# osqp/miosqp

Hardware: AMD Instinct MI355X
Metric: ADMM iterations/s (random_miqp n=500 m=1000 p=250, node-at-a-time B&B) (higher is better)
Workload: dtype f64

## Files before the change

include/miosqp_amd.h:

```cpp
#ifndef MIOSQP_AMD_H
#define MIOSQP_AMD_H

#include <stdint.h>

#ifdef __cplusplus
extern "C" {
#endif

#define MIOSQP_QP_SOLVED 1
#define MIOSQP_QP_MAX_ITER_REACHED (-2)
#define MIOSQP_QP_PRIMAL_INFEASIBLE (-3)
#define MIOSQP_QP_DUAL_INFEASIBLE (-4)
#define MIOSQP_QP_UNSOLVED (-10)

#define MIOSQP_EARG (-1)
#define MIOSQP_EHIP (-2)
#define MIOSQP_EFACTOR (-3)
#define MIOSQP_ENODEV (-4)
#define MIOSQP_EUNSUPPORTED (-5)
#define MIOSQP_EFULL (-6)
#define MIOSQP_EBOUNDS 1

typedef struct miosqp_qp_settings {
  double rho;
// ... 430 lines not shown
                                         double *x_out, miosqp_tree_info *info, miosqp_lockstep_stats *stats,
                                         miosqp_lockstep_ahead_stats *ahead_stats);

typedef struct miosqp_search_info {
  int64_t nodes;
  int64_t osqp_iter;
  int32_t open_leaves;
  int32_t free_slots;
  int32_t improved;
  int32_t reserved;
  double upper_glob, lower_glob;
  double device_time;
  double run_time;
} miosqp_search_info;

int miosqp_qp_search_create(miosqp_qp_engine *e, int32_t capacity);
int miosqp_qp_search_reset(miosqp_qp_engine *e);
int miosqp_qp_search_add_leaf(miosqp_qp_engine *e, const double *l_int, const double *u_int, const double *x0,
                              const double *y0, int32_t depth, double lower);
int miosqp_qp_search_take_leaf(miosqp_qp_engine *e, double *l_int, double *u_int, double *x0, double *y0,
                               int32_t *depth, double *lower);
int miosqp_qp_search_set_incumbent(miosqp_qp_engine *e, double upper, const double *x);
int miosqp_qp_search_get_incumbent(miosqp_qp_engine *e, double *upper, double *x);
int miosqp_qp_search_run(miosqp_qp_engine *e, int32_t tree_explor_rule, int64_t max_nodes, double budget_s,
                         miosqp_search_info *info);

typedef struct miosqp_pool_digest {
  int32_t slot;
  int32_t status_val;
  int32_t iter;
  int32_t int_inf;
  int32_t nextvar;
  int32_t reserved;
  double lower;
  double heur_viol;
  double heur_obj;
  double pri_res, dua_res;
} miosqp_pool_digest;

int miosqp_qp_pool_create(miosqp_qp_engine *e, int32_t capacity, int32_t columns);
int miosqp_qp_pool_reset(miosqp_qp_engine *e);
int miosqp_qp_pool_write_node(miosqp_qp_engine *e, int32_t slot, const double *l_int, const double *u_int,
                              const double *x0, const double *y0);
int miosqp_qp_pool_read_node(miosqp_qp_engine *e, int32_t slot, double *l_int, double *u_int, double *x, double *y);
int miosqp_qp_pool_push(miosqp_qp_engine *e, int32_t count, const int32_t *slot, const int32_t *child0,
                        const int32_t *child1, const double *lower);
// ... 66 lines not shown
```

miosqp_amd/_lib.py:

```python
import ctypes as C
import os

_PKG = os.path.dirname(os.path.abspath(__file__))
LIB_PATH = os.path.join(_PKG, "libmiosqp_hip.so")

dp = C.POINTER(C.c_double)
dpp = C.POINTER(dp)
ip = C.POINTER(C.c_int32)
i64p = C.POINTER(C.c_int64)


class Settings(C.Structure):
    _fields_ = [(k, C.c_double) for k in
                ("rho", "sigma", "alpha", "eps_abs", "eps_rel", "eps_prim_inf", "eps_dual_inf")] + \
               [(k, C.c_int32) for k in ("max_iter", "scaling", "check_termination", "warm_start",
                                         "device", "max_batch", "fold", "resident", "setup_on_device", "coop", "pers", "batch_pers",
                                         "rho_auto")]


class Info(C.Structure):
    _fields_ = [("status_val", C.c_int32), ("iter", C.c_int32), ("run_time", C.c_double),
                ("obj_val", C.c_double), ("pri_res", C.c_double), ("dua_res", C.c_double),
                ("device_time", C.c_double), ("lower", C.c_double),
                ("int_inf", C.c_int32), ("nextvar", C.c_int32), ("heur_viol", C.c_double),
# ... 189 lines not shown
    "miosqp_qp_setup_group": (C.c_int64, [C.c_void_p]),
    "miosqp_qp_debug_product_form": (C.c_int, [C.c_void_p, C.c_int32, dp, C.c_int64, ip, ip]),
    "miosqp_qp_solve_trees_lockstep": (C.c_int, [C.c_void_p, C.c_int32, dp, dp, dp, dp, dp, dp, dp, C.c_int32, C.c_int32,
                                                 C.c_int32, dp, C.POINTER(TreeInfo), C.POINTER(LockstepStats)]),
    "miosqp_qp_solve_trees_lockstep_rf": (C.c_int, [C.c_void_p, C.c_int32, dp, dp, dp, dp, dp, dp, dp, C.c_int32, C.c_int32,
                                                    C.c_int32, C.c_int32, C.c_int32, C.c_int32, dp, C.POINTER(TreeInfo),
                                                    C.POINTER(LockstepStats), C.POINTER(LockstepRfStats)]),
    "miosqp_qp_solve_trees_lockstep_sb": (C.c_int, [C.c_void_p, C.c_int32, dp, dp, dp, dp, dp, dp, dp, C.c_int32, C.c_int32,
                                                    C.c_int32, C.c_int32, C.c_int32, C.c_int32, C.c_int32, C.c_double, dp,
                                                    C.POINTER(TreeInfo), C.POINTER(LockstepStats),
                                                    C.POINTER(LockstepSbStats)]),
    "miosqp_qp_solve_trees_lockstep_ahead": (C.c_int, [C.c_void_p, C.c_int32, dp, dp, dp, dp, dp, dp, dp, C.c_int32,
                                                       C.c_int32, C.c_int32, C.c_int32, dp, C.POINTER(TreeInfo),
                                                       C.POINTER(LockstepStats), C.POINTER(LockstepAheadStats)]),
    "miosqp_qp_solve_trees_refill": (C.c_int, [C.c_void_p, C.c_int32, dp, dp, dp, dp, dp, dp, dp, C.c_int32, C.c_int32,
                                               C.c_int32, dp, C.POINTER(TreeInfo), C.POINTER(RefillStats)]),
    "miosqp_qp_search_create": (C.c_int, [C.c_void_p, C.c_int32]),
    "miosqp_qp_search_reset": (C.c_int, [C.c_void_p]),
    "miosqp_qp_search_add_leaf": (C.c_int, [C.c_void_p, dp, dp, dp, dp, C.c_int32, C.c_double]),
    "miosqp_qp_search_take_leaf": (C.c_int, [C.c_void_p, dp, dp, dp, dp, C.POINTER(C.c_int32), C.POINTER(C.c_double)]),
    "miosqp_qp_search_set_incumbent": (C.c_int, [C.c_void_p, C.c_double, dp]),
    "miosqp_qp_search_get_incumbent": (C.c_int, [C.c_void_p, C.POINTER(C.c_double), dp]),
    "miosqp_qp_search_run": (C.c_int, [C.c_void_p, C.c_int32, C.c_int64, C.c_double, C.POINTER(SearchInfo)]),
    "miosqp_qp_stream_create": (C.c_int, [C.c_void_p, C.c_int32, C.c_int32, C.c_int32]),
    "miosqp_qp_stream_begin": (C.c_int, [C.c_void_p]),
    "miosqp_qp_stream_add_leaf": (C.c_int, [C.c_void_p, dp, dp, dp, dp, C.c_int32, C.c_double]),
    "miosqp_qp_stream_take_leaf": (C.c_int, [C.c_void_p, dp, dp, dp, dp, C.POINTER(C.c_int32), C.POINTER(C.c_double)]),
    "miosqp_qp_stream_set_incumbent": (C.c_int, [C.c_void_p, C.c_double, dp]),
    "miosqp_qp_stream_get_incumbent": (C.c_int, [C.c_void_p, C.POINTER(C.c_double), dp]),
    "miosqp_qp_stream_step": (C.c_int, [C.c_void_p, C.c_int32, C.c_int32, C.c_int32, C.c_int64, C.POINTER(StreamInfo)]),
    "miosqp_qp_solve_batch": (C.c_int, [C.c_void_p, C.c_int32, dp, dp, dp, dp, dp, dp,
                                        C.POINTER(Info)]),
    "miosqp_qp_solve_batch_q": (C.c_int, [C.c_void_p, C.c_int32, dp, dp, dp, dp, dp, dp, dp,
                                          C.POINTER(Info)]),
    "miosqp_qp_solve_tree": (C.c_int, [C.c_void_p, dp, dp, dp, dp, C.c_double, dp, C.c_int32, C.c_int32, dp,
                                       C.POINTER(TreeInfo)]),
    "miosqp_qp_pool_create": (C.c_int, [C.c_void_p, C.c_int32, C.c_int32]),
    "miosqp_qp_pool_reset": (C.c_int, [C.c_void_p]),
    "miosqp_qp_pool_write_node": (C.c_int, [C.c_void_p, C.c_int32, dp, dp, dp, dp]),
    "miosqp_qp_pool_read_node": (C.c_int, [C.c_void_p, C.c_int32, dp, dp, dp, dp]),
    "miosqp_qp_pool_push": (C.c_int, [C.c_void_p, C.c_int32, ip, ip, ip, dp]),
    "miosqp_qp_pool_set_upper": (C.c_int, [C.c_void_p, C.c_double]),
    "miosqp_qp_pool_launch": (C.c_int, [C.c_void_p, C.c_int32]),
    "miosqp_qp_pool_collect": (C.c_int, [C.c_void_p, C.c_int32, C.POINTER(PoolDigest), C.c_int32, C.POINTER(C.c_int32),
                                         C.POINTER(C.c_int32), i64p]),
    "miosqp_qp_cleanup": (C.c_int, [C.c_void_p]),
# ... 61 lines not shown
```

miosqp_amd/csrc/engine.hip:

```cpp
#include <hip/hip_runtime.h>

#include <dlfcn.h>
#include <sys/stat.h>

#include <algorithm>
#include <chrono>
#include <cmath>
#include <cstdio>
#include <cstdlib>
#include <cstring>
#include <map>
#include <mutex>
#include <queue>
#include <deque>
#include <tuple>
#include <type_traits>
#include <string>
#include <vector>

#include "../../include/miosqp_amd.h"
#include "factor.hpp"
#include "polish_many.hpp"
#include "polish_many_large.hpp"
#include "lockstep_trees.hpp"
// ... 76 lines not shown
  double *sm, *sn;
  double *raw_l, *raw_u, *raw_x, *raw_y, *out_x, *out_y;
  Ctrl *ctrl;
  const double *f_rows, *f_GmT, *f_Ad, *f_Atd, *f_Pd;
  int ldf, ldn, ldm;
  double *rx;
  double *xi, *xis, *root_l, *root_u;
  double eps_int, eps_lin;
  int digest;
  int bm_ablate;
  unsigned long long *prof;
  const double *W;
  int ldw;
  unsigned *coop_tag;
  unsigned long long *coop_buf;
  unsigned long long *coop_chk;
  unsigned long long *coop_q;
  unsigned long long *coop_reg;
  unsigned long long *coop_chz;
  unsigned long long *coop_dec;
  int coop_nt;
  int coop_lag;
  int coop_tres;
  const double *Kc;
  int coop_dbg;
  int coop_nap;
  int coop_stride;
  size_t coop_half;
  const double *coop_W;
  int coop_ldw, coop_mg;
  const int *coop_brow;
  const double *coop_aj;
  int Bs;
  double *b_l, *b_u, *b_x, *b_z, *b_y, *b_wh, *b_rx, *b_cv, *b_ut, *b_xt, *b_dx, *b_dy;
  double *b_xfs;
  double *b_sm, *b_sn;
  double *b_xfin, *b_yfin;
  double *b_xi, *b_xis;
  double *b_part;
  const double *b_zero;
  int stream;
  int max_iter_s, ring;
  int *c_start, *c_child0, *c_child1, *c_harv, *t_has;
  int *fmap, *hmap;
  double *lt_x;
  const int *int_pos;
// ... 2573 lines not shown
```

miosqp_amd/csrc/host.inc:

```
constexpr int POOL_EVENTS = 8;
constexpr int COOP_RETRY = -1000;

inline int pick_tpr(double avg_row) {
  if (avg_row <= 48) return 16;
  if (avg_row <= 192) return 32;
  if (avg_row <= 640) return 64;
  if (avg_row <= 1536) return 128;
  return 256;
}

#define DISPATCH_TPR(tpr, KERNEL, rows, stream, ...)                                              \
  do {                                                                                            \
    switch (tpr) {                                                                                \
      case 16: hipLaunchKernelGGL(KERNEL<16>, dim3(((rows) + 15) / 16), dim3(256), 0, stream, __VA_ARGS__); break;   \
      case 32: hipLaunchKernelGGL(KERNEL<32>, dim3(((rows) + 7) / 8), dim3(256), 0, stream, __VA_ARGS__); break;     \
      case 64: hipLaunchKernelGGL(KERNEL<64>, dim3(((rows) + 3) / 4), dim3(256), 0, stream, __VA_ARGS__); break;     \
      case 128: hipLaunchKernelGGL(KERNEL<128>, dim3(((rows) + 1) / 2), dim3(256), 0, stream, __VA_ARGS__); break;   \
      default: hipLaunchKernelGGL(KERNEL<256>, dim3(rows), dim3(256), 0, stream, __VA_ARGS__); break;                \
    }                                                                                             \
  } while (0)

std::mutex g_capture_mutex;

struct ParkedChunk {
// ... 421 lines not shown
  return 0;
}

int coop_pick_cpt(int NR) { return NR < 1024 ? 2 : NR < 1536 ? 3 : 4; }
bool coop_decision_slot(int NR, int cpt) { return NR + 1 <= 512 * cpt; }
int coop_pick_rw(int NR) {
  (void)NR;
  return 8;
}
int coop_pick_testers(int spare) {
  int nt = spare >= 8 ? std::min(COOP_NT_MAX, spare) : 0;
  if (const char *ev = getenv("MIOSQP_COOP_TESTERS")) nt = std::max(0, std::min(std::min(COOP_NT_MAX, spare), atoi(ev)));
  return nt;
}
void coop_pick_lag(miosqp_qp_engine *e) {
  Dev &d = e->d;
  const int n = e->n, M = e->M, N = n + M, nt = d.coop_nt;
  bool res = nt > 0 && (N % 2) == 0 && N - (M & ~1) <= 128 * COOP_RC_S && M <= COOP_RC_R * nt * 8 && n <= COOP_RV_R * nt * 8 &&
             N <= 128 * COOP_RV_S;
  if (const char *ev = getenv("MIOSQP_COOP_TRES")) res = res && atoi(ev) != 0;
  d.coop_tres = res ? 1 : 0;
  d.coop_lag = res ? 10 : 16;
  if (const char *ev = getenv("MIOSQP_COOP_LAG")) d.coop_lag = std::max(1, atoi(ev));
}

#define COOP_FORMS(X) \
  X(8, 2, 2) X(8, 2, 4) X(8, 3, 4) X(8, 4, 4)
int coop_occupancy(int rw, int cpt, int cptf) {
  int per_cu = 0;
  hipError_t oq = hipErrorInvalidValue;
#define X(RW, CPT, CPTF) \
  if (rw == RW && cpt == CPT && cptf == CPTF) oq = hipOccupancyMaxActiveBlocksPerMultiprocessor(&per_cu, k_coop<512, RW, CPT, CPTF, true>, 512, 0);
  COOP_FORMS(X)
#undef X
  return oq == hipSuccess ? per_cu : 0;
}

void launch_coop(miosqp_qp_engine *e, int max_iter, int check_every, int final_check, const CoopNode *node = nullptr) {
  const Dev &d = e->d;
  CoopNode nd{};
  if (node) nd = *node;
  ChipGuard turn(e);
  const bool tst = d.coop_nt > 0 && (check_every <= 0 || check_every > d.coop_lag);
  const int rw = e->coop_rw, cpt = e->coop_cpt, cptf = e->coop_cptf;
#define X(RW, CPT, CPTF)                                                                                              \
  if (rw == RW && cpt == CPT && cptf == CPTF) {                                                                       \
// ... 1172 lines not shown
```

miosqp_amd/csrc/host_search.inc:

```
namespace {

struct NodeSearch {
  int cap = 0;
  double *lo = nullptr, *hi = nullptr, *x = nullptr, *y = nullptr, *inc_x = nullptr;
  double *own_block = nullptr;
  SearchDigest *dg = nullptr;
  unsigned long long seq = 0;
  hipEvent_t ev[4] = {};
  int ev_slot = 0;
  bool ev_pending = false;
  unsigned long long *stamps = nullptr;
  std::vector<int> stamp_iter;
  CoopRun *run_blk = nullptr;
  CoopRun run_blk_host;
  bool run_blk_sent = false;
  unsigned long long *mail_host = nullptr, *mail_dev = nullptr;
  unsigned long long mtag = 0;
  bool run_live = false;
  hipEvent_t ev_run[2] = {};
  int64_t run_off = 0;
  int run_nap = -1;
  std::vector<int> open;
  std::vector<int> freelist, depth, parent, kids;
  std::vector<char> decided;
  std::vector<double> lower;
  double upper = 1.7e308;
  bool have_inc = false;
  int64_t nodes = 0, iters = 0;
};

NodeSearch *search_of(miosqp_qp_engine *e) { return static_cast<NodeSearch *>(e->search); }
bool getenv_off(const char *name) {
  const char *v = getenv(name);
  return v != nullptr && atoi(v) == 0;
}
// ... 410 lines not shown
  if (!x) {
    if (!S.have_inc) return MIOSQP_EARG;
    S.upper = upper;
    return 0;
  }
  if (!(upper < S.upper)) return 0;
  HIPCHK(hipMemcpyAsync(S.inc_x, x, sizeof(double) * e->n, hipMemcpyHostToDevice, e->stream));
  HIPCHK(hipStreamSynchronize(e->stream));
  S.upper = upper;
  S.have_inc = true;
  search_prune(S);
  return 0;
}

int miosqp_qp_search_get_incumbent(miosqp_qp_engine *e, double *upper, double *x) {
  if (!e || !e->search || !upper || !x) return MIOSQP_EARG;
  ENTER(e);
  NodeSearch &S = *search_of(e);
  *upper = S.upper;
  if (S.have_inc) {
    HIPCHK(hipMemcpyAsync(x, S.inc_x, sizeof(double) * e->n, hipMemcpyDeviceToHost, e->stream));
    HIPCHK(hipStreamSynchronize(e->stream));
  }
  return 0;
}

int miosqp_qp_search_run(miosqp_qp_engine *e, int32_t tree_explor_rule, int64_t max_nodes, double budget_s,
                         miosqp_search_info *info) {
  if (!e || !e->search || !info || tree_explor_rule < 0 || tree_explor_rule > 3) return MIOSQP_EARG;
  ENTER(e);
  NodeSearch &S = *search_of(e);
  const double t0 = wall();
  const size_t n = e->n, M = e->M, p = e->d.n_int;
  const Dev &d = e->d;
  int64_t done = 0, it_sum = 0;
  int improved = 0, rc_full = 0;
  double dev_ms = 0.0;
  if (int rc = run_end(e, S, true, nullptr, nullptr)) return rc;
  while (!S.open.empty() && done < max_nodes) {
    if (budget_s > 0 && done > 0 && wall() - t0 >= budget_s) break;
    if (S.freelist.size() < 2) {
      if (int rc = run_end(e, S, true, &dev_ms, nullptr)) return rc;
      const int rcg = search_grow(e, S);
      if (rcg) {
        rc_full = rcg;
        break;
// ... 141 lines not shown
        HIPCHK(hipEventElapsedTime(&lms, e->evc0, e->evc1));
        e->loop_ms += lms;
        dev_ms += lms;
        if (e->node_ms.size() < (size_t)1 << 20) e->node_ms.push_back(lms);
        e->res_pending = e->loop_pending = false;
      }
      e->loop_iters += g.iter;
      if (e->node_it.size() < (size_t)1 << 20) e->node_it.push_back(g.iter);
      if (!g.pad) break;
      reset_registration(e);
      g_err = "cooperative solver: " + std::string(g.pad == 1 ? "the grid was not co-resident within 100 ms (device shared?)"
                                                               : "exchange timed out") + ", stage " + std::to_string(g.pad);
      if (g.pad != 1) return MIOSQP_EHIP;
      if (S.ev_pending) {
        HIPCHK(hipEventSynchronize(S.ev[2 * S.ev_slot + 1]));
        S.ev_pending = false;
      }
      e->loop_iters -= g.iter;
      if (!e->node_it.empty()) e->node_it.pop_back();
      int rc = leave_coop(e);
      if (rc) return rc;
    }
    if (S.stamps) S.stamp_iter[a.seq % 256] = g.todo ? -1 : g.iter;
    done++;
    S.nodes++;
    S.iters += g.iter;
    it_sum += g.iter;
    bool branch = false;
    const bool ok = g.status == MIOSQP_QP_SOLVED || g.status == MIOSQP_QP_MAX_ITER_REACHED;
    if (ok) {
      S.lower[s] = g.lower;
      if (!(g.lower > S.upper)) {
        if (g.int_inf == 0) {
          S.upper = g.lower;
          S.have_inc = true;
          improved = 1;
          search_prune(S);
        } else {
          if (g.action == 2) {
            S.upper = g.heur_obj;
            S.have_inc = true;
            improved = 2;
            search_prune(S);
          }
          branch = g.branched != 0;
        }
// ... 17 lines not shown
    search_done(S, s);
  }
  if (int rc = run_end(e, S, true, &dev_ms, nullptr)) return rc;
  if (S.ev_pending) {
    float lms = 0;
    HIPCHK(hipEventSynchronize(S.ev[2 * S.ev_slot + 1]));
    HIPCHK(hipEventElapsedTime(&lms, S.ev[2 * S.ev_slot], S.ev[2 * S.ev_slot + 1]));
    e->loop_ms += lms;
    dev_ms += lms;
    if (e->node_ms.size() < (size_t)1 << 20) e->node_ms.push_back(lms);
    S.ev_pending = false;
  }
  if (S.stamps && done > 0) {
    HIPCHK(hipStreamSynchronize(e->stream));
    std::vector<unsigned long long> h(256 * 16);
    HIPCHK(hipMemcpy(h.data(), S.stamps, sizeof(unsigned long long) * h.size(), hipMemcpyDeviceToHost));
    double sum[16] = {};
    double its = 0;
    int cnt = 0;
    for (int k = 0; k < 256; k++) {
      const unsigned long long *w = &h[16 * k];
      if (S.stamp_iter[k] <= 0 || !w[0] || !w[10] || w[10] < w[0]) continue;
      for (int q = 1; q <= 15; q++) sum[q] += 0.01 * (double)((long long)w[q] - (long long)w[0]);
      its += S.stamp_iter[k];
      cnt++;
    }
    if (cnt)
      fprintf(stderr, "[search stamps] %d nodes, %.1f it/node; us after kernel entry: go %.1f  round0 %.1f  tester's test rows %.1f  "
                      "tester gathered %.1f  decision %.1f  grid left loop %.1f  grid wrote back %.1f  epilogue rows %.1f  gathered %.1f  "
                      "record %.1f | tester 0's epilogue: entered %.1f  x built %.1f  rows %.1f  sums+digest %.1f  slot written %.1f\n",
              cnt, its / cnt, sum[1] / cnt, sum[2] / cnt, sum[3] / cnt, sum[4] / cnt, sum[5] / cnt,
              sum[6] / cnt, sum[7] / cnt, sum[8] / cnt, sum[9] / cnt, sum[10] / cnt, sum[13] / cnt, sum[11] / cnt, sum[12] / cnt,
              sum[14] / cnt, sum[15] / cnt);
  }
  info->nodes = done;
  info->osqp_iter = it_sum;
  info->open_leaves = (int32_t)S.open.size();
  info->free_slots = (int32_t)S.freelist.size();
  info->improved = improved;
  info->upper_glob = S.upper;
  double lg = 1.0 / 0.0;
  for (int s2 : S.open) lg = S.lower[s2] < lg ? S.lower[s2] : lg;
  info->lower_glob = S.open.empty() ? S.upper : lg;
  info->device_time = 1e-3 * dev_ms;
  info->run_time = wall() - t0;
  return rc_full;
// ... 4 lines not shown
```

miosqp_amd/csrc/kernels_coop.inc:

```
constexpr unsigned long long COOP_LIMIT_REGISTER = 10000000ull, COOP_LIMIT_EXCHANGE = 200000000ull;
__device__ __forceinline__ bool coop_expired(unsigned &spins, unsigned long long &since,
                                             unsigned long long limit = COOP_LIMIT_EXCHANGE) {
  if ((++spins & 4095u) != 0u) return false;
  const unsigned long long now = wall_clock64();
  if (spins == 4096u) {
    since = now;
    return false;
  }
  return now - since > limit;
}

typedef unsigned ll_u4 __attribute__((ext_vector_type(4)));
__device__ __forceinline__ void ll_publish(unsigned long long *slot, double v, unsigned tag) {
  ll_u4 w;
  w.x = (unsigned)__double2loint(v); w.y = tag; w.z = (unsigned)__double2hiint(v); w.w = tag;
  asm volatile("global_store_dwordx4 %0, %1, off sc1\n\ts_nop 1" ::"v"(slot), "v"(w) : "memory");
}
__device__ __forceinline__ ll_u4 ll_peek(const unsigned long long *slot) {
  ll_u4 w;
  asm volatile("global_load_dwordx4 %0, %1, off sc1" : "=v"(w) : "v"(slot) : "memory");
  return w;
}

constexpr unsigned long long COOP_SENTINEL = 0x7FF0000000005EA7ull;
// ... 385 lines not shown
  __syncthreads();
  return s_status;
}

constexpr int COOP_NT_MAX = 64;
__device__ __forceinline__ double coop_wsum(double v) {
#pragma unroll
  for (int off = 32; off > 0; off >>= 1) v += __shfl_xor(v, off, 64);
  return v;
}

struct CoopTesterArgs {
  unsigned long long *coop_chk, *coop_chz, *coop_q, *coop_dec, *prof;
  const double *Kc, *Einv, *E, *Dinv, *D, *l, *u, *q;
  Ctrl *ctrl;
  int n, M, ldw;
  double c, cinv, eps_abs, eps_rel, eps_pinf, eps_dinf;
  int epi;
  unsigned long long *stamps;
  int res;
  int run;
  unsigned long long *coop_buf, coop_half;
  int NR, lag;
};
#define COOP_STAMP(ptr, k)                                          \
  do {                                                              \
    if ((ptr) != nullptr && threadIdx.x == 0) (ptr)[k] = wall_clock64(); \
  } while (0)

__device__ __forceinline__ double coop_prow(const int *__restrict__ idx, const double *__restrict__ val, int s, int e, int t, int tpr,
                                            const lds_f64 *v) {
  double a0 = 0.0, a1 = 0.0;
  for (int k = s + 2 * t; k < e; k += 2 * tpr) {
    const double2 a = *reinterpret_cast<const double2 *>(val + k);
    const int2 j = *reinterpret_cast<const int2 *>(idx + k);
    a0 = fma(a.x, v[j.x], a0);
    a1 = fma(a.y, v[j.y], a1);
  }
  return a0 + a1;
}
__device__ __forceinline__ void coop_prow2(const int *__restrict__ idx, const double *__restrict__ val, int s, int e, int t, int tpr,
                                           const lds_f64 *v, const lds_f64 *w, double &rv, double &rw) {
  double a0 = 0.0, a1 = 0.0, b0 = 0.0, b1 = 0.0;
  for (int k = s + 2 * t; k < e; k += 2 * tpr) {
    const double2 a = *reinterpret_cast<const double2 *>(val + k);
    const int2 j = *reinterpret_cast<const int2 *>(idx + k);
// ... 71 lines not shown
  REC_ST(t0, t0); REC_ST(t1, (unsigned long long)wall_clock64());
  asm volatile("s_waitcnt vmcnt(0)" ::: "memory");
  REC_ST(seq, seq);
#undef REC_ST
}
template <int COOP_B>
__device__ __attribute__((noinline)) void coop_epi_rows(const CoopEpi *dp, unsigned long long *stamps, const int w, const int G,
                                              const unsigned tag, const double *lv0, double *s1, double *s2, double *red) {
  const CoopEpi &d = *dp;
  const int t = threadIdx.x, n = d.n, M = d.M;
  lds_f64 *const ox = to_lds(s1), *const xi = to_lds(s1) + 1024, *const xis = to_lds(s2);
  const lds_f64 *const lx = to_lds(lv0);
  for (int i = t; i < n; i += COOP_B) {
    double o = d.D[i] * lx[M + i];
    const int k = d.int_pos[i];
    if (k >= 0) o = fmin(fmax(o, epi_ld(d.a.lo_s + k, d.coh)), epi_ld(d.a.hi_s + k, d.coh));
    ox[i] = o;
    const double r = k >= 0 ? rint(o) : o;
    xi[i] = r;
    xis[i] = d.Dinv[i] * r;
  }
  __syncthreads();
  COOP_STAMP(stamps, 11);
  double vmax = -1.7e308;
  const int Gh = COOP_B / d.tpr_h, Go = COOP_B / d.tpr_o;
  const int CH = (M + Gh - 1) / Gh, CO = (n + Go - 1) / Go;
  for (int c = w; c < CH + CO; c += G) {
    if (c < CH) {
      const int tpr = d.tpr_h, g = t / tpr, tr = t % tpr;
      const int row_raw = c * Gh + g;
      const bool live = row_raw < M;
      const int row = live ? row_raw : M - 1;
      const double ei = d.Einv[row], rl = d.root_l[row], ru = d.root_u[row];
      double acc[1];
      acc[0] = coop_prow(d.pc_idx, d.pc_A, d.pc_ptr[row], d.pc_ptr[row + 1], tr, tpr, xis);
      coop_row_reduce<1>(acc, tpr, red);
      if (live && tr == 0) {
        const double z = ei * acc[0];
        vmax = fmax(vmax, fmax(rl - d.eps_lin - z, z - ru - d.eps_lin));
      }
    } else {
      const int tpr = d.tpr_o, g = t / tpr, tr = t % tpr;
      const int row_raw = (c - CH) * Go + g;
      const bool live = row_raw < n;
      const int row = live ? row_raw : n - 1;
      const double qr = d.qraw[row];
// ... 147 lines not shown
    c->heur_viol = hviol;
    const lds_f64 *const rc = to_lds(rec);
    coop_record(d.a.dg, st, it, int_inf, nv, action, branched, lower, hviol, hobj, rc[0], rc[1], rc[2], d.t_node, d.a.seq);
    COOP_STAMP(stamps, 10);
  }
}

constexpr int COOP_RC_R = 3, COOP_RC_S = 4, COOP_RV_R = 1, COOP_RV_S = 16;
template <int COOP_B, int CPTF, bool RES>
__device__ __attribute__((noinline)) void coop_tester(const CoopTesterArgs *dp, const CoopEpi *ep, const int T, const int max_iter,
                                            const int check_every, const int final_check, const unsigned base, int *s_fail,
                                            double *lvp, double *lz) {
  CoopTesterArgs d;
  {
    const auto *l = (const __attribute__((address_space(3))) CoopTesterArgs *)dp;
    d.coop_chk = coop_uni(l->coop_chk); d.coop_chz = coop_uni(l->coop_chz); d.coop_q = coop_uni(l->coop_q);
    d.coop_dec = coop_uni(l->coop_dec); d.prof = coop_uni(l->prof); d.Kc = coop_uni(l->Kc); d.Einv = coop_uni(l->Einv);
    d.E = coop_uni(l->E); d.Dinv = coop_uni(l->Dinv); d.D = coop_uni(l->D); d.l = coop_uni(l->l); d.u = coop_uni(l->u);
    d.q = coop_uni(l->q); d.ctrl = coop_uni(l->ctrl); d.n = coop_uni(l->n); d.M = coop_uni(l->M); d.ldw = coop_uni(l->ldw);
    d.c = coop_uni(l->c); d.cinv = coop_uni(l->cinv); d.eps_abs = coop_uni(l->eps_abs); d.eps_rel = coop_uni(l->eps_rel);
    d.eps_pinf = coop_uni(l->eps_pinf); d.eps_dinf = coop_uni(l->eps_dinf); d.epi = coop_uni(l->epi);
    d.stamps = coop_uni(l->stamps); d.res = coop_uni(l->res); d.run = coop_uni(l->run);
    d.coop_buf = coop_uni(l->coop_buf); d.coop_half = coop_uni(l->coop_half); d.NR = coop_uni(l->NR); d.lag = coop_uni(l->lag);
  }
  constexpr int NW = COOP_B / 64;
  lds_f64 *const lv0 = to_lds(lvp), *const lv1 = to_lds(lvp) + 2048, *const lzl = to_lds(lz);
  __shared__ double qw[NW][NQ];
  __shared__ double qall[COOP_NT_MAX * NQ];
  __shared__ double qres[NQ];
  __shared__ int s_status;
  __shared__ double s_rec[3];
  const int t = threadIdx.x, lane = t & 63, wave = t >> 6;
  const int M = d.M, N = d.n + d.M;
  const int j = (int)blockIdx.x - T, NT = (int)gridDim.x - T;
  const double NEUTRAL = -1.7e308;
  const int Ne = N & ~1;
  auto rows_load = [&](auto RC, auto SC, const bool con, const int first, const int step, const int end, auto &a, auto &sc_inv,
                       auto &sc_dir, auto &lo, auto &up, auto &qv) {
    constexpr int R = decltype(RC)::value, S = decltype(SC)::value;
    const int cbeg = (con ? (M & ~1) : 0) + 2 * lane;
#pragma unroll
    for (int i = 0; i < R; i++) {
      const int rr = first + i * step;
      const int rc = rr < end ? rr : end - 1;
      const double *row = d.Kc + (size_t)rc * d.ldw;
#pragma unroll
// ... 227 lines not shown
        rows_apply(integral_constant<int, COOP_RC_R>{}, integral_constant<int, COOP_RC_S>{}, true, fc, step, M, rca, s_rsc[wave][0],
                   s_rsc[wave][1], s_rsc[wave][2], s_rsc[wave][3], s_rsc[wave][4], acc);
        rows_apply(integral_constant<int, COOP_RV_R>{}, integral_constant<int, COOP_RV_S>{}, false, fv, step, N, rva, s_rsv[wave][0],
                   s_rsv[wave][1], s_rsv[wave][2], s_rsv[wave][3], s_rsv[wave][4], acc);
      } else {
      const int n_cols = N - (M & ~1);
      if (n_cols <= 512) batch(integral_constant<int, 6>{}, integral_constant<int, 4>{}, true, fc, step, M);
      else if (n_cols <= 1024) batch(integral_constant<int, 3>{}, integral_constant<int, 8>{}, true, fc, step, M);
      else batch(integral_constant<int, 2>{}, integral_constant<int, 16>{}, true, fc, step, M);
      if (N <= 1024) batch(integral_constant<int, 4>{}, integral_constant<int, 8>{}, false, fv, step, N);
      else batch(integral_constant<int, 2>{}, integral_constant<int, 16>{}, false, fv, step, N);
      }
    }
    if (lane < NQ) qw[wave][lane] = acc;
    if (stamp) st[2] = wall_clock64();
    __syncthreads();
    if (j == 0) COOP_STAMP(d.stamps, 3);
    if (stamp) st[3] = wall_clock64();
    if (t < NQ) {
      double rq = qw[0][t];
      for (int w = 1; w < NW; w++) rq = t < NQ_MAX ? fmax(rq, qw[w][t]) : rq + qw[w][t];
      ll_publish(d.coop_q + (size_t)j * COOP_QS + 2 * t, rq, tag);
    }
    if (j == 0) {
      {
        constexpr int KC = (COOP_NT_MAX * NQ + COOP_B - 1) / COOP_B;
        const int ne = NT * NQ;
        bool have[KC];
#pragma unroll
        for (int k = 0; k < KC; k++) have[k] = t + k * COOP_B >= ne;
        unsigned spins = 0;
        unsigned long long since = 0;
        static_assert(KC == 3, "ll_peek_waitn<3>");
        for (;;) {
          const unsigned long long *ptr[KC];
          ll_u4 w[KC];
#pragma unroll
          for (int k = 0; k < KC; k++) {
            const int e0 = t + k * COOP_B;
            ptr[k] = d.coop_q + (have[k] ? 0 : (size_t)(e0 / NQ) * COOP_QS + 2 * (e0 % NQ));
          }
          ll_peek_waitn<KC>(ptr, w);
          bool all = true;
#pragma unroll
          for (int k = 0; k < KC; k++) {
            if (have[k]) continue;
// ... 57 lines not shown
            s_status = (int)__hiloint2double((int)w.z, (int)w.x);
            break;
          }
          if (coop_expired(spins, since)) {
            *s_fail = 1;
            d.ctrl->pad = 10;
            s_status = -1;
            break;
          }
          __builtin_amdgcn_s_sleep(4);
        }
      }
      __syncthreads();
    }
    if (stamp) st[4] = wall_clock64();
    if (*s_fail) return;
    {
      const int stn = s_status;
      const bool last = final_check && it == max_iter;
      if (d.epi && (stn == MIOSQP_QP_SOLVED || (stn == 0 && last))) {
        __syncthreads();
        unsigned long long *const stp = j == 0 ? d.stamps : nullptr;
        COOP_STAMP(stp, 13);
        coop_epi_rows<COOP_B>(ep, stp, (int)blockIdx.x, (int)gridDim.x, tag, lvp, lvp + 2048, lz, &qw[0][0]);
        if (j == 0)
          coop_epi_commit<COOP_B>(ep, stp, (int)gridDim.x, tag, stn == 0 ? MIOSQP_QP_MAX_ITER_REACHED : stn, it, lvp, lvp + 2048, lz,
                                  &qw[0][0], s_rec, s_fail);
        return;
      }
      if (d.epi && stn != 0) {
        if (j == 0 && t == 0) {
          Ctrl *c = d.ctrl;
          const double nan = __builtin_nan("");
          c->int_inf = -1;
          c->nextvar = -1;
          c->lower = c->heur_obj = c->heur_viol = nan;
          coop_record(ep->a.dg, stn, it, -1, -1, 0, 0, nan, nan, nan, s_rec[0], s_rec[1], s_rec[2], ep->t_node, ep->a.seq);
          COOP_STAMP(d.stamps, 10);
        }
        return;
      }
    }
    if (s_status) return;
    __syncthreads();
  }
}

__device__ __forceinline__ void coop_register(unsigned long long *reg, Ctrl *ctrl, int *s_fail) {
  *s_fail = 0;
  const unsigned G = gridDim.x;
// ... 128 lines not shown
  a.lo0 = (double *)s_mail[CM_LO0]; a.hi0 = (double *)s_mail[CM_HI0];
  a.lo1 = (double *)s_mail[CM_LO1]; a.hi1 = (double *)s_mail[CM_HI1];
  a.inc_x = blk->inc_x;
  a.upper = __longlong_as_double((long long)s_mail[CM_UPPER]);
  a.dg = blk->dg;
  a.seq = s_mail[CM_SEQ];
  nd->epi_buf = blk->epi_buf;
  nd->stamps = (unsigned long long *)s_mail[CM_STAMPS];
}

template <class DV, class NV>
__device__ __forceinline__ void coop_fill_epi(CoopEpi *ep, const DV &d, const NV &nd, const int coh) {
  *ep = CoopEpi{d.D, d.Dinv, d.E, d.Einv, d.pc_A, d.pr_val, d.qraw, d.root_l, d.root_u, d.int_pos, d.i_idx,
                d.pc_ptr, d.pc_idx, d.pr_ptr, d.pr_idx, d.ctrl, d.n, d.M, d.n_int, nd.tpr_h, nd.tpr_o, d.cinv,
                d.eps_int, d.eps_lin, SearchArgs{nd.a.lo_s, nd.a.hi_s, nd.a.x_w, nd.a.y_w, nd.a.x_s, nd.a.y_s, nd.a.lo0, nd.a.hi0,
                                                 nd.a.lo1, nd.a.hi1, nd.a.inc_x, nd.a.upper, nd.a.dg, nd.a.seq},
                nd.epi_buf, nullptr, coh, (unsigned long long)wall_clock64()};
}
template <class DV, class NV>
__device__ __forceinline__ void coop_fill_tester(CoopTesterArgs *ta, const DV &d, const NV &nd, const int run) {
  *ta = CoopTesterArgs{d.coop_chk, d.coop_chz, d.coop_q, d.coop_dec, d.prof, d.Kc, d.Einv, d.E, d.Dinv, d.D, d.l,
                       d.u, d.q, d.ctrl, d.n, d.M, d.ldw, d.c, d.cinv, d.eps_abs, d.eps_rel,
                       d.eps_pinf, d.eps_dinf, nd.on && nd.epi, nd.on ? nd.stamps : nullptr, d.coop_tres, run,
                       d.coop_buf, (unsigned long long)d.coop_half, d.coop_mg + d.n, d.coop_lag};
}
__device__ __forceinline__ void coop_ctrl_reset(Ctrl *c) {
  c->done = 0;
  c->pad = 0;
  c->status = MIOSQP_QP_UNSOLVED;
  c->iter = 0;
  c->pri_res = c->dua_res = c->obj_val = 0.0;
  c->lower = __builtin_nan("");
}

template <int RW, int NW, bool TST>
struct CoopLds {
  __attribute__((aligned(16))) double part[2][RW][NW];
  double s_ko[RW][6];
  __attribute__((aligned(16))) double lvs[TST ? 2 * 2048 : 2];
  __attribute__((aligned(16))) double lzs[TST ? COOP_EPI_ENTRIES : 2];
  CoopTesterArgs s_ta;
  CoopEpi s_ep;
  __attribute__((aligned(8))) int s_fail;
  int s_dec;
  unsigned long long s_mail[CM_WORDS];
  CoopNode s_nd;
};
// ... 348 lines not shown
      if (dv) {
        status = dv;
        if (own) { o.z = s_ko[t][0]; o.y = s_ko[t][1]; o.dy = s_ko[t][2]; o.sw = s_ko[t][3]; o.x = s_ko[t][4]; o.dx = s_ko[t][5]; }
        it_rep = last;
      }
    }
  }
  GRID_STAMP(6);
  if (it > max_iter) it = max_iter;
  const int it_done = it;
  if (it_rep >= 0) it = it_rep;
  if (prof && t == 0) {
    unsigned long long *out = d.prof + 8 * blockIdx.x;
    out[0] = ph0; out[1] = ph1; out[2] = ph2; out[3] = it; out[4] = ph3; out[5] = ph4; out[6] = nchk; out[7] = ph5;
  }
  if (own && !called_off) {
    if (con) { d.z[o.rowc] = o.z; d.y[o.rowc] = o.y; d.dy[o.rowc] = o.dy; d.wh[o.rowc] = o.sw; }
    if (var) { d.x[o.var] = o.x; d.dx[o.var] = o.dx; d.rx[o.var] = sigma * o.x - o.q; }
  }
  GRID_STAMP(7);
  const bool epi_here = TST && nd.on && nd.epi && !called_off && !s_fail &&
                        (status == MIOSQP_QP_SOLVED || (status == 0 && final_check && it_rep < 0));
  const bool rec_here = epi_here || (TST && nd.on && nd.epi && !called_off && !s_fail && status != 0);
  if constexpr (TST) {
    if (epi_here) {
      if (t == 0) fill_epi();
      const unsigned etag = base + 1u + (unsigned)it;
      const int n = d.n;
      for (int i0 = 0; i0 < n; i0 += COOP_B) {
        const int i = i0 + t;
        const unsigned long long *ptr = d.coop_chk + 4 * (size_t)(M + (i < n ? i : 0));
        unsigned spins = 0;
        unsigned long long since = 0;
        for (;;) {
          const ll_u4 w = ll_peek_wait(ptr);
          if (w.y == etag && w.w == etag) {
            if (i < n) lvs[M + i] = __hiloint2double((int)w.z, (int)w.x);
            break;
          }
          if (coop_expired(spins, since)) {
            d.ctrl->pad = 13;
            break;
          }
        }
      }
      __syncthreads();
      coop_epi_rows<COOP_B>(&s_ep, nullptr, (int)blockIdx.x, (int)gridDim.x, etag, lvs, lvs + 2048, lzs, &part[0][0][0]);
    }
// ... 144 lines not shown
```

miosqp_amd/qp.py:

```python
import ctypes as C
import types

import numpy as np
import scipy.sparse as spa

from miosqp_amd import _lib

_ALIASES = {"eps_inf": "eps_prim_inf", "eps_unb": "eps_dual_inf",
            "early_terminate_interval": "check_termination"}
_IGNORED = {"verbose", "polish", "polishing", "linsys_solver", "time_limit", "scaled_termination",
            "delta", "polish_refine_iter", "early_terminate"}


def constant(name):
    v = _lib.load().miosqp_qp_constant(name.encode())
    if v == 0:
        raise ValueError("Constant %s not found" % name)
    return v


def default_settings():
    s = _lib.Settings()
    _lib.load().miosqp_qp_default_settings(C.byref(s))
    return s
# ... 789 lines not shown
            self._h, _vec(l_int, k, "l_int"), _vec(u_int, k, "u_int"), _vec(x0, self.n, "x0"), _vec(y0, self.m, "y0"),
            int(depth), float(lower)), "search_add_leaf")
        if rc == 1:
            raise ValueError("Lower bound must be lower than or equal to upper bound")

    def search_take_leaf(self, n_int, into=None):
        l, u, x, y = into if into is not None else (np.empty(n_int), np.empty(n_int), np.empty(self.n), np.empty(self.m))
        depth, lower = C.c_int32(), C.c_double()
        rc = _check(self._lib.miosqp_qp_search_take_leaf(self._h, _vec(l, n_int, "l_int"), _vec(u, n_int, "u_int"),
                                                         _vec(x, self.n, "x0"), _vec(y, self.m, "y0"),
                                                         C.byref(depth), C.byref(lower)), "search_take_leaf")
        return None if rc == 1 else (l, u, x, y, depth.value, lower.value)

    def search_set_incumbent(self, upper, x):
        _check(self._lib.miosqp_qp_search_set_incumbent(self._h, float(upper),
                                                        None if x is None else _lib.as_d(_f64(x, self.n, "x"))),
               "search_set_incumbent")

    def search_get_incumbent(self):
        upper, x = C.c_double(), np.empty(self.n)
        _check(self._lib.miosqp_qp_search_get_incumbent(self._h, C.byref(upper), _lib.as_d(x)), "search_get_incumbent")
        return (upper.value, x) if upper.value < 1.7e308 else (float("inf"), None)

    def search_run(self, tree_explor_rule, max_nodes, budget_s=0.0):
        info = self._search_info
        max_nodes = 2 ** 62 if not np.isfinite(max_nodes) else int(min(int(max_nodes), 2 ** 62))
        rc = self._lib.miosqp_qp_search_run(self._h, int(tree_explor_rule), max_nodes, float(budget_s), C.byref(info))
        info.full = rc == -6
        if not info.full:
            _check(rc, "search_run")
        return info

    def stream_create(self, capacity, columns, ring_margin=0):
        _check(self._lib.miosqp_qp_stream_create(self._h, int(capacity), int(columns), int(ring_margin)), "stream_create")
        self._stream_info = _lib.StreamInfo()

    def stream_begin(self):
        _check(self._lib.miosqp_qp_stream_begin(self._h), "stream_begin")

    def stream_add_leaf(self, l_int, u_int, x0, y0, depth, lower):
        k = len(l_int)
        rc = _check(self._lib.miosqp_qp_stream_add_leaf(
            self._h, _vec(l_int, k, "l_int"), _vec(u_int, k, "u_int"), _vec(x0, self.n, "x0"), _vec(y0, self.m, "y0"),
            int(depth), float(lower)), "stream_add_leaf")
        if rc == 1:
            raise ValueError("Lower bound must be lower than or equal to upper bound")
# ... 213 lines not shown
```

Measured before the change: 597,100.

## Speculatively run epilogue rows on tester blocks during cooperative termination check

Adds a speculative epilogue mode, on by default when there are at least two tester blocks. Non-leader tester blocks compute their share of the epilogue rows right after publishing the termination reduction, instead of waiting for the solved decision. The leader block then commits, and the worker-side epilogue wait is skipped. This aims to take the epilogue off the critical path after convergence, at the cost of wasted work on iterations that do not terminate. It also adds a per-node search log API and an extra timing stamp sum for profiling.

```diff
diff --git a/include/miosqp_amd.h b/include/miosqp_amd.h
--- a/include/miosqp_amd.h
+++ b/include/miosqp_amd.h
@@ -476,6 +476,8 @@
                                int32_t *depth, double *lower);
 int miosqp_qp_search_set_incumbent(miosqp_qp_engine *e, double upper, const double *x);
 int miosqp_qp_search_get_incumbent(miosqp_qp_engine *e, double *upper, double *x);
+int miosqp_qp_search_set_node_log(miosqp_qp_engine *e, int32_t capacity);
+int miosqp_qp_search_get_node_log(miosqp_qp_engine *e, int32_t max_nodes, int32_t *ints, double *lower, int32_t *count);
 int miosqp_qp_search_run(miosqp_qp_engine *e, int32_t tree_explor_rule, int64_t max_nodes, double budget_s,
                          miosqp_search_info *info);
 
diff --git a/miosqp_amd/_lib.py b/miosqp_amd/_lib.py
--- a/miosqp_amd/_lib.py
+++ b/miosqp_amd/_lib.py
@@ -235,6 +235,8 @@
     "miosqp_qp_search_set_incumbent": (C.c_int, [C.c_void_p, C.c_double, dp]),
     "miosqp_qp_search_get_incumbent": (C.c_int, [C.c_void_p, C.POINTER(C.c_double), dp]),
     "miosqp_qp_search_run": (C.c_int, [C.c_void_p, C.c_int32, C.c_int64, C.c_double, C.POINTER(SearchInfo)]),
+    "miosqp_qp_search_set_node_log": (C.c_int, [C.c_void_p, C.c_int32]),
+    "miosqp_qp_search_get_node_log": (C.c_int, [C.c_void_p, C.c_int32, C.POINTER(C.c_int32), dp, C.POINTER(C.c_int32)]),
     "miosqp_qp_stream_create": (C.c_int, [C.c_void_p, C.c_int32, C.c_int32, C.c_int32]),
     "miosqp_qp_stream_begin": (C.c_int, [C.c_void_p]),
     "miosqp_qp_stream_add_leaf": (C.c_int, [C.c_void_p, dp, dp, dp, dp, C.c_int32, C.c_double]),
diff --git a/miosqp_amd/csrc/engine.hip b/miosqp_amd/csrc/engine.hip
--- a/miosqp_amd/csrc/engine.hip
+++ b/miosqp_amd/csrc/engine.hip
@@ -122,6 +122,7 @@
   int coop_nt;
   int coop_lag;
   int coop_tres;
+  int coop_spec;
   const double *Kc;
   int coop_dbg;
   int coop_nap;
diff --git a/miosqp_amd/csrc/host.inc b/miosqp_amd/csrc/host.inc
--- a/miosqp_amd/csrc/host.inc
+++ b/miosqp_amd/csrc/host.inc
@@ -467,6 +467,8 @@
   d.coop_tres = res ? 1 : 0;
   d.coop_lag = res ? 10 : 16;
   if (const char *ev = getenv("MIOSQP_COOP_LAG")) d.coop_lag = std::max(1, atoi(ev));
+  d.coop_spec = nt >= 2 ? 1 : 0;
+  if (const char *ev = getenv("MIOSQP_COOP_EPI_SPEC")) d.coop_spec = d.coop_spec && atoi(ev) != 0;
 }
 
 #define COOP_FORMS(X) \
diff --git a/miosqp_amd/csrc/host_search.inc b/miosqp_amd/csrc/host_search.inc
--- a/miosqp_amd/csrc/host_search.inc
+++ b/miosqp_amd/csrc/host_search.inc
@@ -11,6 +11,8 @@
   bool ev_pending = false;
   unsigned long long *stamps = nullptr;
   std::vector<int> stamp_iter;
+  std::vector<SearchDigest> log;
+  size_t log_cap = 0;
   CoopRun *run_blk = nullptr;
   CoopRun run_blk_host;
   bool run_blk_sent = false;
@@ -467,6 +469,28 @@
     HIPCHK(hipMemcpyAsync(x, S.inc_x, sizeof(double) * e->n, hipMemcpyDeviceToHost, e->stream));
     HIPCHK(hipStreamSynchronize(e->stream));
   }
+  return 0;
+}
+
+int miosqp_qp_search_set_node_log(miosqp_qp_engine *e, int32_t capacity) {
+  if (!e || !e->search || capacity < 0) return MIOSQP_EARG;
+  NodeSearch &S = *search_of(e);
+  S.log.clear();
+  S.log_cap = (size_t)capacity;
+  return 0;
+}
+
+int miosqp_qp_search_get_node_log(miosqp_qp_engine *e, int32_t max_nodes, int32_t *ints, double *lower, int32_t *count) {
+  if (!e || !e->search || max_nodes < 0 || !ints || !lower || !count) return MIOSQP_EARG;
+  NodeSearch &S = *search_of(e);
+  const size_t k = std::min(S.log.size(), (size_t)max_nodes);
+  for (size_t i = 0; i < k; i++) {
+    const SearchDigest &g = S.log[i];
+    const int32_t v[5] = {g.status, g.iter, g.nextvar, g.action, g.branched};
+    memcpy(ints + 5 * i, v, sizeof(v));
+    lower[i] = g.lower;
+  }
+  *count = (int32_t)k;
   return 0;
 }
 
@@ -654,6 +678,7 @@
       if (rc) return rc;
     }
     if (S.stamps) S.stamp_iter[a.seq % 256] = g.todo ? -1 : g.iter;
+    if (S.log.size() < S.log_cap) S.log.push_back(g);
     done++;
     S.nodes++;
     S.iters += g.iter;
@@ -717,6 +742,7 @@
       const unsigned long long *w = &h[16 * k];
       if (S.stamp_iter[k] <= 0 || !w[0] || !w[10] || w[10] < w[0]) continue;
       for (int q = 1; q <= 15; q++) sum[q] += 0.01 * (double)((long long)w[q] - (long long)w[0]);
+      if (w[12] > w[8]) sum[8] += 0.01 * (double)((long long)w[12] - (long long)w[8]);
       its += S.stamp_iter[k];
       cnt++;
     }
diff --git a/miosqp_amd/csrc/kernels_coop.inc b/miosqp_amd/csrc/kernels_coop.inc
--- a/miosqp_amd/csrc/kernels_coop.inc
+++ b/miosqp_amd/csrc/kernels_coop.inc
@@ -431,6 +431,7 @@
   int run;
   unsigned long long *coop_buf, coop_half;
   int NR, lag;
+  int spec;
 };
 #define COOP_STAMP(ptr, k)                                          \
   do {                                                              \
@@ -548,6 +549,7 @@
   }
   __syncthreads();
   COOP_STAMP(stamps, 11);
+  if (w < 0) return;
   double vmax = -1.7e308;
   const int Gh = COOP_B / d.tpr_h, Go = COOP_B / d.tpr_o;
   const int CH = (M + Gh - 1) / Gh, CO = (n + Go - 1) / Go;
@@ -741,6 +743,7 @@
     d.eps_pinf = coop_uni(l->eps_pinf); d.eps_dinf = coop_uni(l->eps_dinf); d.epi = coop_uni(l->epi);
     d.stamps = coop_uni(l->stamps); d.res = coop_uni(l->res); d.run = coop_uni(l->run);
     d.coop_buf = coop_uni(l->coop_buf); d.coop_half = coop_uni(l->coop_half); d.NR = coop_uni(l->NR); d.lag = coop_uni(l->lag);
+    d.spec = coop_uni(l->spec);
   }
   constexpr int NW = COOP_B / 64;
   lds_f64 *const lv0 = to_lds(lvp), *const lv1 = to_lds(lvp) + 2048, *const lzl = to_lds(lz);
@@ -1014,6 +1017,11 @@
       for (int w = 1; w < NW; w++) rq = t < NQ_MAX ? fmax(rq, qw[w][t]) : rq + qw[w][t];
       ll_publish(d.coop_q + (size_t)j * COOP_QS + 2 * t, rq, tag);
     }
+    const bool spec = d.spec && NT >= 2 && !(final_check && it == max_iter);
+    if (spec && j != 0) {
+      __syncthreads();
+      coop_epi_rows<COOP_B>(ep, j == 1 ? d.stamps : nullptr, j - 1, NT - 1, tag, lvp, lvp + 2048, lz, &qw[0][0]);
+    }
     if (j == 0) {
       {
         constexpr int KC = (COOP_NT_MAX * NQ + COOP_B - 1) / COOP_B;
@@ -1117,10 +1125,11 @@
         __syncthreads();
         unsigned long long *const stp = j == 0 ? d.stamps : nullptr;
         COOP_STAMP(stp, 13);
-        coop_epi_rows<COOP_B>(ep, stp, (int)blockIdx.x, (int)gridDim.x, tag, lvp, lvp + 2048, lz, &qw[0][0]);
+        if (!spec) coop_epi_rows<COOP_B>(ep, stp, (int)blockIdx.x, (int)gridDim.x, tag, lvp, lvp + 2048, lz, &qw[0][0]);
+        else if (j == 0) coop_epi_rows<COOP_B>(ep, stp, -1, NT - 1, tag, lvp, lvp + 2048, lz, &qw[0][0]);
         if (j == 0)
-          coop_epi_commit<COOP_B>(ep, stp, (int)gridDim.x, tag, stn == 0 ? MIOSQP_QP_MAX_ITER_REACHED : stn, it, lvp, lvp + 2048, lz,
-                                  &qw[0][0], s_rec, s_fail);
+          coop_epi_commit<COOP_B>(ep, stp, spec ? NT - 1 : (int)gridDim.x, tag, stn == 0 ? MIOSQP_QP_MAX_ITER_REACHED : stn, it, lvp,
+                                  lvp + 2048, lz, &qw[0][0], s_rec, s_fail);
         return;
       }
       if (d.epi && stn != 0) {
@@ -1295,7 +1304,8 @@
   *ta = CoopTesterArgs{d.coop_chk, d.coop_chz, d.coop_q, d.coop_dec, d.prof, d.Kc, d.Einv, d.E, d.Dinv, d.D, d.l,
                        d.u, d.q, d.ctrl, d.n, d.M, d.ldw, d.c, d.cinv, d.eps_abs, d.eps_rel,
                        d.eps_pinf, d.eps_dinf, nd.on && nd.epi, nd.on ? nd.stamps : nullptr, d.coop_tres, run,
-                       d.coop_buf, (unsigned long long)d.coop_half, d.coop_mg + d.n, d.coop_lag};
+                       d.coop_buf, (unsigned long long)d.coop_half, d.coop_mg + d.n, d.coop_lag,
+                       run && nd.on && nd.epi && d.coop_spec};
 }
 __device__ __forceinline__ void coop_ctrl_reset(Ctrl *c) {
   c->done = 0;
@@ -1690,8 +1700,9 @@
   const bool epi_here = TST && nd.on && nd.epi && !called_off && !s_fail &&
                         (status == MIOSQP_QP_SOLVED || (status == 0 && final_check && it_rep < 0));
   const bool rec_here = epi_here || (TST && nd.on && nd.epi && !called_off && !s_fail && status != 0);
+  const bool epi_spec = RUN && d.coop_spec && d.coop_nt >= 2 && status == MIOSQP_QP_SOLVED && !(final_check && it == max_iter);
   if constexpr (TST) {
-    if (epi_here) {
+    if (epi_here && !epi_spec) {
       if (t == 0) fill_epi();
       const unsigned etag = base + 1u + (unsigned)it;
       const int n = d.n;
diff --git a/miosqp_amd/qp.py b/miosqp_amd/qp.py
--- a/miosqp_amd/qp.py
+++ b/miosqp_amd/qp.py
@@ -835,6 +835,17 @@
         _check(self._lib.miosqp_qp_search_get_incumbent(self._h, C.byref(upper), _lib.as_d(x)), "search_get_incumbent")
         return (upper.value, x) if upper.value < 1.7e308 else (float("inf"), None)
 
+    def search_node_log(self, capacity=None):
+        if capacity is not None:
+            self._node_log_cap = int(capacity)
+            _check(self._lib.miosqp_qp_search_set_node_log(self._h, int(capacity)), "search_set_node_log")
+            return None
+        cap = getattr(self, "_node_log_cap", 0)
+        ints, lower, k = np.zeros((max(cap, 1), 5), dtype=np.int32), np.zeros(max(cap, 1)), C.c_int32()
+        _check(self._lib.miosqp_qp_search_get_node_log(self._h, cap, ints.ctypes.data_as(C.POINTER(C.c_int32)), _lib.as_d(lower),
+                                                       C.byref(k)), "search_get_node_log")
+        return ints[:k.value].copy(), lower[:k.value].copy()
+
     def search_run(self, tree_explor_rule, max_nodes, budget_s=0.0):
         info = self._search_info
         max_nodes = 2 ** 62 if not np.isfinite(max_nodes) else int(min(int(max_nodes), 2 ** 62))
```

Result: no change. 595,000 (-0.3%).
